# templeblock/audioSignalProcess

Hardware: AMD Instinct MI355X
Metric: audio frames/sec (10 ms @16 kHz) Wiener NS (higher is better)
Workload: dtype f32

## Files before the change

### audiosignalprocess_amd/csrc/ns_kernels1.hip

```cpp
#include <hip/hip_runtime.h>

#include <type_traits>

#include "handoff.h"
#include "ns_device.h"
#include "ns_layout.h"
#include "ns_pair_fft.h"
#include "ns_step.h"

namespace {
using namespace asphandoff;
using namespace aspns_dev;
using namespace aspns_pair;

__device__ __forceinline__ unsigned long long ns_cu_tag() {
  const unsigned hw = __builtin_amdgcn_s_getreg((7 << 11) | (8 << 6) | 4);
  const unsigned xcc = __builtin_amdgcn_s_getreg((3 << 11) | (0 << 6) | 20);
  return (unsigned long long)((xcc << 8) | hw);
}

constexpr int NS3 = 3;

template <typename V>
__device__ __forceinline__ V ns_in_vgpr(V x) {
// ... 98 lines not shown
  }
  __device__ __forceinline__ void image_fill(int lane, const float4 (&v)[kImgVec4]) const {
#pragma unroll
    for (int i = 0; i < kImgVec4; ++i)
      *reinterpret_cast<lds_f32x4*>(img + i * 256 + 4 * lane) = f32x4v{v[i].x, v[i].y, v[i].z, v[i].w};
  }
  __device__ __forceinline__ void image_write_back(int lane) const {
#pragma unroll
    for (int i = 0; i < kImgVec4; ++i) {
      const f32x4v v = *reinterpret_cast<const lds_f32x4*>(img + i * 256 + 4 * lane);
      sc1_store4(rs, lane * 16, i * 1024, make_float4(v.x, v.y, v.z, v.w));
    }
  }
};

template <bool IMG>
struct ScalarRow {
  lds_f32* row;
  static constexpr int kTrk0 = aspns::S_TAIL0 + aspns::V_LQ0, kTrk1 = aspns::S_TAIL0 + aspns::V_DEN2;
  static constexpr bool in_image(int k) { return IMG && k >= aspns::S_OVERDRIVE && !(k >= kTrk0 && k <= kTrk1); }
  __device__ __forceinline__ explicit ScalarRow(float* image) : row((lds_f32*)image + aspns::kOffScalars) {}
  template <int K>
  __device__ __forceinline__ float f(float sv) const {
    if constexpr (in_image(K)) return row[K];
    else return __int_as_float(__builtin_amdgcn_readlane(__float_as_int(sv), K));
  }
  template <int K, int N>
  __device__ __forceinline__ void ld(float sv, float (&v)[N]) const {
    static_assert((N == 2 || N == 4) && K % N == 0 && in_image(K) == in_image(K + N - 1), "one aligned group, one master");
    if constexpr (in_image(K) && N == 2) {
      const f32x2v t = *reinterpret_cast<const lds_f32x2*>(row + K);
      v[0] = t.x; v[1] = t.y;
    } else if constexpr (in_image(K)) {
      const f32x4v t = *reinterpret_cast<const lds_f32x4*>(row + K);
      v[0] = t.x; v[1] = t.y; v[2] = t.z; v[3] = t.w;
    } else {
#pragma unroll
      for (int i = 0; i < N; ++i) v[i] = __int_as_float(__builtin_amdgcn_readlane(__float_as_int(sv), K + i));
    }
  }
  template <int K>
  __device__ __forceinline__ void set(float& sv, float val) const {
    if constexpr (in_image(K)) row[K] = val;
    else sv = setlane_vgpr<K>(sv, val);
  }
  __device__ __forceinline__ void store_owned(int lane, float sv) const {
    if (!IMG || lane < aspns::S_OVERDRIVE || (lane >= kTrk0 && lane <= kTrk1)) row[lane] = sv;
  }
};

struct NsStepScalars {
  int blockInd;
  int updates;
  int counter[3];
  int updateParsFlag;
  int mup3;
  int gainmap;
};
#define NS_STEADY_CONJUNCTS(X, s)                                                                                   \
  X((s).blockInd > NS_END_STARTUP_LONG + 1)                                           \
  X((s).updates >= NS_END_STARTUP_LONG)                                                                              \
  X((s).counter[0] < NS_END_STARTUP_LONG - 1 && (s).counter[1] < NS_END_STARTUP_LONG - 1 &&                           \
    (s).counter[2] < NS_END_STARTUP_LONG - 1)                               \
  X((s).counter[0] >= 0 && (s).counter[1] >= 0 && (s).counter[2] >= 0)                                                \
  X((s).updateParsFlag >= 1)                                                                                         \
  X((s).mup3 > 2)                                                                \
  X((s).gainmap == 1)
__device__ __forceinline__ bool ns_step_is_steady(const NsStepScalars& s) {
  bool steady = true;
#define NS_CONJ_AND(c) steady = steady && (c);
  NS_STEADY_CONJUNCTS(NS_CONJ_AND, s)
#undef NS_CONJ_AND
  return steady;
}
__device__ __forceinline__ void ns_assume_steady(const NsStepScalars& s) {
#define NS_CONJ_ASSUME(c) __builtin_assume(c);
  NS_STEADY_CONJUNCTS(NS_CONJ_ASSUME, s)
#undef NS_CONJ_ASSUME
}

struct NsDiagArgs {
  void* buf;
  int mode;
};

template <bool IO16, bool FLOW, bool DIAG>
__device__ __forceinline__ void ns_frame1_run(float* __restrict__ state, int32_t* __restrict__ hist_all,
                                              const NsTables* __restrict__ T, const float* __restrict__ in,
                                              float* __restrict__ out, int num_streams, int steady_on,
                                              const NsFlowArgs& fa, const NsDiagArgs& dg) {
  [[maybe_unused]] const unsigned long long diag_buf =
      DIAG ? (FLOW ? ns_in_vgpr((unsigned long long)dg.buf) : (unsigned long long)dg.buf) : 0ull;
#ifdef NS1_BUDGET
#define NS_STAMP(k) asm volatile("; NS_PHASE " #k " body %0" : : "n"(ns_body_tag));
#define NS_BUDGET_ASIDE() asm volatile("; NS_PHASE 99 body 3");
#define NS_BUDGET_BACK(k) asm volatile("; NS_PHASE " #k " body %0" : : "n"(ns_body_tag));
#else
  [[maybe_unused]] unsigned stamp_sel = 0;
  if constexpr (DIAG) {
    if (dg.buf != nullptr && dg.mode != 2 && threadIdx.x < 64) {
      if (dg.mode == 1) stamp_sel = 1u;
      else if (FLOW ? blockIdx.x == gridDim.x / 2 : blockIdx.x == 0) stamp_sel = 2u + (FLOW ? fa.steps / 2 : 0u);
    }
  }
#define NS_STAMP(k)                                                                            \
  if constexpr (DIAG) {                                                                        \
    const unsigned stamp_sel_ = __builtin_amdgcn_readfirstlane(stamp_sel);                     \
    if (stamp_sel_ != 0) {                                                                     \
      __builtin_amdgcn_sched_barrier(0);                                                       \
      unsigned long long* const stamps_ = reinterpret_cast<unsigned long long*>(diag_buf);     \
      if (stamp_sel_ == 1u) {                                                                  \
        if ((k) == 0 || (k) == 1 || (k) == 14 || (k) == 15)                                    \
          stamps_[blockIdx.x * 4 + ((k) == 0 ? 0 : (k) == 1 ? 1 : (k) == 14 ? 2 : 3)] =       \
              __builtin_amdgcn_s_memrealtime() | ((k) == 0 ? ns_cu_tag() << 48 : 0ull);       \
      } else if (stamp_sel_ == 2u + flow_j) {                                                  \
        stamps_[k] = __builtin_amdgcn_s_memtime();                                             \
      }                                                                                        \
      __builtin_amdgcn_sched_barrier(0);                                                       \
    }                                                                                          \
  }
#define NS_BUDGET_ASIDE()
#define NS_BUDGET_BACK(k)
#endif
  unsigned flow_j = 0, flow_end = 1, flow_slot = 0;
  [[maybe_unused]] unsigned diag_steps = 0;
  [[maybe_unused]] constexpr int ns_body_tag = 0;
  if constexpr (FLOW) {
    flow_j = blockIdx.y * fa.walk;
    flow_end = flow_j + fa.walk < fa.steps ? flow_j + fa.walk : fa.steps;
    flow_slot = ((unsigned)fa.slot0 + flow_j) % (unsigned)fa.ring;
  } else {
    NS_STAMP(0)
  }
  __shared__ __align__(16) float2 lds[4][130];
  __shared__ __align__(16) float tabs[3 * 64 * 4 + 32 * 4 * 2];
  __shared__ __align__(16) float wins[kAnal];
  __shared__ __align__(16) double exp2s[64];
  __shared__ __align__(16) double2 logts[128];
  __shared__ __align__(16) float imgs[FLOW ? 4 : 1][FLOW ? kImgDwords : 4];
  const int tid = threadIdx.x;
  const float4* tab_src = tid < 192 ? reinterpret_cast<const float4*>(&T->tw[0][0][0]) + tid
                                    : reinterpret_cast<const float4*>(&T->spl[0][0][0]) + (tid - 192);
  const float4 tab_v = *tab_src;
  const float4 win_v = reinterpret_cast<const float4*>(T->window)[tid & 63];
  const double exp2_v = T->exp2_64[tid & 63];
  const double2 logt_v = reinterpret_cast<const double2*>(T->logtab)[tid & 127];
  const int lane = tid & 63;
  const int diagbits = T->diag[lane];
  const int wv = __builtin_amdgcn_readfirstlane(tid >> 6);
  float2* tile = lds[wv];
  const int lam = lane >> 1, h = lane & 1;
  const int g = lam >> 4, q = lam & 15;
  const int binA = q + 64 * g + 16 * h;
  const uint32_t gmask = g ? 0x80000000u : 0u;
  const int stream_raw = blockIdx.x * 4 + wv;
  bool wave_live = stream_raw < num_streams;
  const int stream = wave_live ? stream_raw : num_streams - 1;
  float* __restrict__ st = state + (size_t)stream * kStreamDwords;
  int32_t* __restrict__ hist = hist_all + (size_t)stream * kHistDwords;
  const StateAcc<FLOW> sa(st, FLOW ? imgs[wv] : nullptr);
  float* outj = out;
  auto diag_flush_steps = [&]() __attribute__((always_inline)) {
    if constexpr (DIAG) {
      unsigned* const counts = reinterpret_cast<unsigned*>(diag_buf);
      if (dg.mode == 2 && ns_cold(lane) == 0) {
        atomicAdd(counts + 2 * stream, diag_steps & 0xffffu);
        atomicAdd(counts + 2 * stream + 1, diag_steps >> 16);
      }
    }
  };

  float sv;
  constexpr bool ROW_IMG = FLOW && !DIAG;
  const ScalarRow<ROW_IMG> srow(imgs[FLOW ? wv : 0]);
#define SC_I(k) __builtin_amdgcn_readlane(__float_as_int(sv), (k))
#define SC_F(k) srow.template f<(k)>(sv)
#define SC_SET_I(k, val) sv = writelane_bits<(k)>(sv, (int)(val))
#define SC_SET_F(k, val) srow.template set<(k)>(sv, (val))
  static_assert(S_COUNTER1 == S_COUNTER0 + 1 && S_COUNTER2 == S_COUNTER0 + 2, "the three counters: consecutive lanes");
  float4 s4;
  float2 carryA, carryB;
  float4 s4in = make_float4(0.f, 0.f, 0.f, 0.f);
  const size_t frame_uni = (size_t)stream * kBlockL;
  auto flow_load_in = [&](unsigned slot) __attribute__((always_inline)) {
    const int lane_c = ns_cold(lane);
    const unsigned frame_lane = 4u * (unsigned)((lane_c < 24 ? 24 : lane_c) - 24);
    const float* base = IO16 ? reinterpret_cast<const float*>(reinterpret_cast<const short*>(in + (size_t)slot * fa.per) + frame_uni)
                             : in + (size_t)slot * fa.per + frame_uni;
    s4in = load_frame4<IO16>(base, frame_lane);
  };
  auto flow_head = [&](auto head_c) __attribute__((always_inline)) {
    [[maybe_unused]] constexpr int ns_body_tag = decltype(head_c)::value;
    NS_STAMP(0)
    outj = out + (size_t)flow_slot * fa.per;
    const int lane_c = ns_cold(lane);
    const float4 ha = sa.ld4(kOffAnaHist, 4 * (lane_c < 24 ? lane_c : 23));
    const bool hsel = lane_c < 24;
    s4.x = hsel ? ha.x : s4in.x;
    s4.y = hsel ? ha.y : s4in.y;
    s4.z = hsel ? ha.z : s4in.z;
    s4.w = hsel ? ha.w : s4in.w;
    const int q2_c = lane_c & 30;
    carryA = sa.ld2(kOffSynt, q2_c + 32 * (lane_c & 1));
    carryB = sa.ld2(kOffSynt, q2_c + 64);
  };
  [[maybe_unused]] float4 img_v[FLOW ? kImgVec4 : 1];
  if constexpr (FLOW) {
    flow_load_in(flow_slot);
    if (wave_live) wave_live = handoff_wait(fa.hand, fa.want + flow_j, stream, lane);
    if (wave_live) sa.image_request(lane, img_v);
  } else {
    sv = st[kOffScalars + lane];
    float* hbuf = st + kOffAnaHist;
    if (!IO16) {
      const float* src = lane < 24 ? hbuf + 4 * lane : in + (size_t)stream * kBlockL + 4 * (lane - 24);
      s4 = *reinterpret_cast<const float4*>(src);
    } else {
      const int lh = lane < 24 ? lane : 23, li = lane < 24 ? 24 : lane;
      const float4 ha = *reinterpret_cast<const float4*>(hbuf + 4 * lh);
      const short* in16 = reinterpret_cast<const short*>(in) + (size_t)stream * kBlockL + 4 * (li - 24);
      const short4 a = *reinterpret_cast<const short4*>(in16);
      const bool hsel = lane < 24;
      s4.x = hsel ? ha.x : (float)a.x;
      s4.y = hsel ? ha.y : (float)a.y;
      s4.z = hsel ? ha.z : (float)a.z;
      s4.w = hsel ? ha.w : (float)a.w;
    }
    carryA = *reinterpret_cast<const float2*>(st + kOffSynt + 2 * q + 32 * h);
    carryB = *reinterpret_cast<const float2*>(st + kOffSynt + 2 * q + 64);
  }

  reinterpret_cast<float4*>(tabs)[tid] = tab_v;
  if (tid < 64) exp2s[tid] = exp2_v;
  if (tid < 128) logts[tid] = logt_v;
  if (tid >= 192) reinterpret_cast<float4*>(wins)[tid - 192] = win_v;
  if constexpr (FLOW) {
    if (wave_live) sa.image_fill(lane, img_v);
  }
  __syncthreads();
  if (!wave_live) return;
  if constexpr (FLOW) {
    sv = sa.ld1(kOffScalars, lane);
    flow_head(std::integral_constant<int, 3>{});
  }
  const float* tws = tabs;
  const float* spls = tabs + 3 * 64 * 4;
  const PairFftLane fl = pair_fft_lane(lane, diagbits);

#define LOADV(dst, f)                                                                          \
  {                                                                                            \
    const float2 v2_ = sa.ld2(kOffVec + (f)*kVecStride, 2 * lane);                             \
    dst[0] = v2_.x; dst[1] = v2_.y;                                                            \
  }
#define LOADT(dst, f) dst[2] = SC_F(S_TAIL0 + (f));
#define LOAD3(dst, f) LOADV(dst, f) LOADT(dst, f)
#define STORE3(f, srcv)                                                                        \
  {                                                                                            \
    sa.st2(kOffVec + (f)*kVecStride, 2 * lane, srcv[0], srcv[1]);                              \
    SC_SET_F(S_TAIL0 + (f), srcv[2]);                                                          \
  }
#define STORE3_HOT(f, srcv)                                                                    \
  {                                                                                            \
    sa.st2(kOffVec + (f)*kVecStride, 2 * lane, srcv[0], srcv[1]);                              \
    if constexpr (!ROW_IMG) SC_SET_F(S_TAIL0 + (f), srcv[2]);                                  \
  }
#define NS_NEXT_FRAME()                                                                        \
  if constexpr (FLOW) {                                                                        \
    flow_slot = flow_slot + 1u == (unsigned)fa.ring ? 0u : flow_slot + 1u;                     \
    if (flow_j + 1u < flow_end) flow_load_in(flow_slot);                                       \
  }
#define NS_STREAM_DONE(head_tag)                                                               \
  if constexpr (FLOW) {                                                                        \
    [[maybe_unused]] constexpr int ns_body_tag = head_tag;  \
    const bool walk_done_ = flow_j + 1u >= flow_end;                                           \
    if (walk_done_) {                                                                          \
      NS_BUDGET_ASIDE()                                                                        \
      const int lane_w_ = ns_cold(lane);                                                       \
      srow.store_owned(lane_w_, sv);                                                           \
      lds_sync1();                                                                             \
      sa.image_write_back(lane_w_);                                                            \
      handoff_drain();                                                                         \
    }                                                                                          \
    NS_STAMP(16)                                                                               \
    if (walk_done_) {                                                                          \
      NS_BUDGET_ASIDE()                                                                        \
      diag_flush_steps();                                                                      \
      if (lane == 0) handoff_publish(fa.hand.seq + stream, fa.want + flow_j);                  \
      return;                                                                                  \
    }                                                                                          \
    ++flow_j;                                                                                  \
    lds_sync1();                                                                               \
    NS_BUDGET_BACK(16)                                                                         \
    flow_head(std::integral_constant<int, head_tag>{});                                        \
    continue;                                                                                  \
  } else {                                                                                     \
    diag_flush_steps();                                                                        \
    return;                                                                                    \
  }

  constexpr bool CARRY = FLOW;
  [[maybe_unused]] f32x2 carry_stsa = {0.f, 0.f};
  [[maybe_unused]] float carry_stsa_tail = 0.f;
  [[maybe_unused]] bool carry_ok = false;
  for (;;) {
    NS_BUDGET_BACK(0)
    float LQ[3][NS3], DEN[3][NS3], quant[NS3];
    float smooth[NS3], noisePrev[NS3], magnPrevA[NS3], logLrt[NS3], avgPause[NS3];


    const float4 w4 = *reinterpret_cast<const float4*>(wins + 4 * lane);
    const float wx0 = w4.x * s4.x, wx1 = w4.y * s4.y, wx2 = w4.z * s4.z, wx3 = w4.w * s4.w;
    float epart = wx0 * wx0;
    epart += wx1 * wx1;
    epart += wx2 * wx2;
    epart += wx3 * wx3;
    const float energy1 = wave_sum_bcast(epart);

    {
      const int lane_c = ns_cold(lane);
      if (lane_c >= 40) sa.st4(kOffAnaHist, 4 * (lane_c - 40), s4);
    }

    if (energy1 == 0.0f) {
      NS_BUDGET_ASIDE()
      float* y = IO16 ? reinterpret_cast<float*>(reinterpret_cast<short*>(outj) + (size_t)stream * kBlockL)
                      : outj + (size_t)stream * kBlockL;
      NS_NEXT_FRAME()
      const int lane_c = ns_cold(lane);
      float2 o01 = make_float2(0.f, 0.f);
      if (lane_c < 48) o01 = sa.ld2(kOffSynt, 2 * lane_c);
      __builtin_amdgcn_fence(__ATOMIC_ACQ_REL, "wavefront");
      store2p<IO16>(y, 2 * lane_c, sat16p(o01.x), sat16p(o01.y));
      if (lane_c < 16) store2p<IO16>(y, 128 + 2 * lane_c, 0.f, 0.f);
      if (lane_c < 48) sa.st2(kOffSynt, 2 * lane_c, 0.f, 0.f);
      NS_STREAM_DONE(3)
    }
    NS_BUDGET_BACK(0)

    LOADV(LQ[0], V_LQ0) LOADV(LQ[1], V_LQ1) LOADV(LQ[2], V_LQ2)
    LOADV(DEN[0], V_DEN0) LOADV(DEN[1], V_DEN1) LOADV(DEN[2], V_DEN2)
    LOADV(quant, V_QUANT)
    NS_STAMP(1)
    *reinterpret_cast<float4*>(&tile[2 * lane]) = make_float4(wx0, wx1, wx2, wx3);
    lds_sync1();
    f32x2 er, ei;
    {
      f32x2 ea, eb;
      cft128_passes1(tile, tws, fl, lane, ea, eb);
      radix2_tail1(ea, eb, gmask, false, er, ei);
    }
    real_split1(tile, spls, lane, er, ei, false);

    NS_STAMP(2)
    if constexpr (!CARRY) LOADV(magnPrevA, V_MAGNPREV_A)
    LOADV(logLrt, V_LOGLRT) LOADV(avgPause, V_AVGPAUSE)
    if constexpr (!CARRY) LOADV(smooth, V_SMOOTH)
    LOADV(noisePrev, V_NOISEPREV)

    float re[NS3], im[NS3], magn[NS3];
    re[0] = er.x;
    im[0] = ei.x;
    re[1] = er.y;
    im[1] = ei.y;
    re[2] = lane_bcast(ei.x, 0);
    im[2] = 0.f;
    if (lane == 0) im[0] = 0.f;
    {
      float m2[2] = {re[0] * re[0] + im[0] * im[0], re[1] * re[1] + im[1] * im[1]}, rt[2];
      fsqrt_n<2>(m2, rt);
      magn[0] = rt[0] + 1.f;
      magn[1] = rt[1] + 1.f;
    }
    if (lane == 0) magn[0] = fabsf(re[0]) + 1.f;
    magn[2] = fabsf(re[2]) + 1.f;

#define SUM3(v) (wave_sum_bcast(v[0] + v[1]) + v[2])

    NsStepScalars ss;
    ss.blockInd = SC_I(S_BLOCKIND) + 1;
    ss.updates = SC_I(S_UPDATES);
    ss.counter[0] = SC_I(S_COUNTER0);
    ss.counter[1] = SC_I(S_COUNTER1);
    ss.counter[2] = SC_I(S_COUNTER2);
    ss.updateParsFlag = SC_I(S_MUP0);
    ss.mup3 = SC_I(S_MUP3);
    ss.gainmap = SC_I(S_GAINMAP);
    const bool step_steady = steady_on != 0 && ns_step_is_steady(ss);
    static_assert(kCntTerms == NS_END_STARTUP_LONG + 1, "one entry per counter value");
    float cterm[3][3];
    auto load_cterms = [&]() __attribute__((always_inline)) {
#pragma unroll
      for (int s = 0; s < 3; ++s) {
        typedef const __attribute__((address_space(4))) float cfloat_k;
        const unsigned n = (unsigned)ss.counter[s] < (unsigned)NS_END_STARTUP_LONG ? (unsigned)ss.counter[s]
                                                                                   : (unsigned)NS_END_STARTUP_LONG;
#pragma unroll
        for (int j = 0; j < 3; ++j) cterm[s][j] = *(cfloat_k*)(&T->cnt_terms[n][j]);
      }
    };
    auto step_rest = [&](auto steady_c) __attribute__((always_inline)) {
      constexpr bool STEADY = decltype(steady_c)::value;
      [[maybe_unused]] constexpr int ns_body_tag = STEADY ? 1 : 2;
      if constexpr (STEADY) ns_assume_steady(ss);
      if constexpr (DIAG) diag_steps += STEADY ? 1u : 0x10000u;
      load_cterms();
      const int blockInd = ss.blockInd;
      float priorSpeechProb;
      const int gainmap = ss.gainmap;

      float noise[NS3], prevStsa[NS3];
      const int updateParsFlag = ss.updateParsFlag;
      int updates = ss.updates;
      int counter[3] = {ss.counter[0], ss.counter[1], ss.counter[2]};

      float snrLocPost[NS3], snrLocPrior[NS3];
      auto snr_tail = [&](float noise2) __attribute__((always_inline)) {
        const float q2t = fdiv(magn[2], noise2 + 0.0001f);
        float previousEstimateStsa;
        if (CARRY && carry_ok) {
          previousEstimateStsa = carry_stsa_tail;
        } else {
          const float q1t = fdiv(magnPrevA[2], noisePrev[2] + 0.0001f);
          previousEstimateStsa = q1t * smooth[2];
        }
        prevStsa[2] = previousEstimateStsa;
        snrLocPost[2] = 0.f;
        if (magn[2] > noise2) snrLocPost[2] = q2t - 1.f;
        snrLocPrior[2] = NS_DD_PR_SNR * previousEstimateStsa + (1.f - NS_DD_PR_SNR) * snrLocPost[2];
      };
      auto load_snr_tails = [&]() __attribute__((always_inline)) {
        static_assert(V_SMOOTH == V_QUANT + 1 && V_MAGNPREV_A == V_NOISEPREV + 1, "row tails read as pairs");
        float t2[2], u2[2];
        srow.template ld<S_TAIL0 + V_QUANT, 2>(sv, t2);
        srow.template ld<S_TAIL0 + V_NOISEPREV, 2>(sv, u2);
        quant[2] = t2[0]; smooth[2] = t2[1];
        noisePrev[2] = u2[0]; magnPrevA[2] = u2[1];
      };
      float lmagn[NS3];
      [[maybe_unused]] float lt1_tail = 0.f;
      if constexpr (STEADY) {
        load_snr_tails();
        snr_tail(quant[2]);
        const float xs[NS3] = {magn[0], magn[1], lane == 1 ? 1.f + 2.f * snrLocPrior[2] : magn[2]};
        log_f32_via_tab_n<NS3>(xs, lmagn, logts);
        lt1_tail = lane_bcast(lmagn[2], 1);
        lmagn[2] = lane_bcast(lmagn[2], 0);
      } else {
        log_f32_via_tab_n<NS3>(magn, lmagn, logts);
      }
      LOADT(avgPause, V_AVGPAUSE)

      NS_STAMP(3)
      float signalEnergy, sumMagn, flatNum, avgPauseMean;
      {
        float p_se = (re[0] * re[0] + im[0] * im[0]) + (re[1] * re[1] + im[1] * im[1]);
        float p_sm = magn[0] + magn[1];
        float p_fl = lane == 0 ? lmagn[1] : lmagn[0] + lmagn[1];
        float p_ap = avgPause[0] + avgPause[1];
        wave_sums_bcast(p_se, p_sm, p_fl, p_ap);
        signalEnergy = p_se + (re[2] * re[2] + im[2] * im[2]);
        sumMagn = p_sm + magn[2];
        flatNum = p_fl + lmagn[2];
        avgPauseMean = p_ap + avgPause[2];
        signalEnergy = DIV129(signalEnergy);
      }

      NS_STAMP(4)
      if constexpr (!STEADY) load_snr_tails();
      if (updates < NS_END_STARTUP_LONG) updates++;
      bool quant_new = false;
      constexpr int kLqLane = S_TAIL0 + V_LQ0, kDenLane = S_TAIL0 + V_DEN0;
      static_assert(V_LQ1 == V_LQ0 + 1 && V_LQ2 == V_LQ0 + 2 && V_DEN1 == V_DEN0 + 1 && V_DEN2 == V_DEN0 + 2 &&
                    kDenLane == kLqLane + 3 && kLqLane / 16 == (kDenLane + 2) / 16,
                    "the tracker tails: three + three consecutive lanes of one DPP row");
      float lqT = sv, denT = dpp_move<0x103>(sv);
      {
#define NS_LANES3_F(j) __int_as_float(lanes3_bits<kLqLane>(__float_as_int(cterm[0][j]), __float_as_int(cterm[1][j]), \
                                                           __float_as_int(cterm[2][j])))
        const float cntv = NS_LANES3_F(0), cnt1v = NS_LANES3_F(1), rcnt1v = NS_LANES3_F(2);
#undef NS_LANES3_F
        tracker_step1(lqT, denT, lmagn[2], cntv, cnt1v, rcnt1v);
      }
#pragma unroll
      for (int s = 0; s < 3; ++s) {
        {
          const float cnt = cterm[s][0], cnt1 = cterm[s][1], rcnt1 = cterm[s][2];
          f32x2 lq = {LQ[s][0], LQ[s][1]}, den = {DEN[s][0], DEN[s][1]};
          tracker_step2(lq, den, f32x2{lmagn[0], lmagn[1]}, cnt, cnt1, rcnt1);
          LQ[s][0] = lq.x; LQ[s][1] = lq.y;
          DEN[s][0] = den.x; DEN[s][1] = den.y;
        }
        if (counter[s] >= NS_END_STARTUP_LONG) {
          counter[s] = 0;
          if (updates >= NS_END_STARTUP_LONG) {
            LQ[s][2] = lane_bcast(lqT, kLqLane + s);
            exp_f32_via_f64_n<NS3>(LQ[s], quant, exp2s);
            quant_new = true;
          }
        }
        counter[s]++;
      }
      if (updates < NS_END_STARTUP_LONG) {
        LQ[2][2] = lane_bcast(lqT, kLqLane + 2);
        exp_f32_via_f64_n<NS3>(LQ[2], quant, exp2s);
        quant_new = true;
      }
#pragma unroll
      for (int k = 0; k < NS3; ++k) noise[k] = quant[k];
#pragma unroll
      for (int s = 0; s < 3; ++s) sa.st2(kOffVec + (V_LQ0 + s) * kVecStride, 2 * lane, LQ[s][0], LQ[s][1]);
#pragma unroll
      for (int s = 0; s < 3; ++s) sa.st2(kOffVec + (V_DEN0 + s) * kVecStride, 2 * lane, DEN[s][0], DEN[s][1]);
      sv = mergelanes_vgpr<(7ull << kLqLane)>(sv, lqT);
      sv = mergelanes_vgpr<(7ull << kDenLane)>(sv, dpp_move<0x113>(denT));
      if (quant_new) STORE3(V_QUANT, quant)

      NS_STAMP(5)
// ... 211 lines not shown
        priorSpeechProb = ns_prior_update(priorSpeechProb, pm, ns_prior_indicator(lane_bcast(th, 0)),
                                          ns_prior_indicator(lane_bcast(th, 1)), ns_prior_indicator(lane_bcast(th, 2)));
      }
      float probSpeech[NS3];
      {
        const float gainPrior = fdiv(1.f - priorSpeechProb, priorSpeechProb + 0.0001f);
        {
          float pd[NS3];
          const float ones[NS3] = {1.f, 1.f, 1.f};
#pragma unroll
          for (int k = 0; k < NS3; ++k) {
            float invLrt = ev[k];
            invLrt = (float)gainPrior * invLrt;
            pd[k] = 1.f + invLrt;
          }
          fdiv3(ones, pd, probSpeech);
        }
      }

      NS_STAMP(10)
      {
        const int srcA = q > 0 ? lane - 2 : (h ? 30 + 32 * g : 31);
        const int srcB = q > 0 ? lane - 2 : (h ? 30 + 32 * g : 31 + 32 * g);
        const bool a_from1 = q == 0 && h == 0;
        const bool b_from1 = q > 0 || h == 1;
        const float a0 = __shfl(probSpeech[0], srcA, 64), a1 = __shfl(probSpeech[1], srcA, 64);
        const float b0 = __shfl(probSpeech[0], srcB, 64), b1 = __shfl(probSpeech[1], srcB, 64);
        float prevProb[NS3];
        prevProb[0] = a_from1 ? a1 : a0;
        prevProb[1] = b_from1 ? b1 : b0;
        prevProb[2] = lane_bcast(probSpeech[1], 63);
        {
          const F3 np(noisePrev), mg(magn), ps(probSpeech), ap(avgPause);
          const F3 x = (1.f - ps) * mg + ps * np;
          const F3 uS = NS_SPEECH_UPDATE * np + (1.f - NS_SPEECH_UPDATE) * x;
          const F3 uN = NS_NOISE_UPDATE * np + (1.f - NS_NOISE_UPDATE) * x;
          B3 oldSpeech = gt3(F3(prevProb), F3(NS_PROB_RANGE));
          oldSpeech.v[0] = oldSpeech.v[0] && lane != 0;
          const F3 uOld = sel3(oldSpeech, uS, uN);
          const F3 uNew = sel3(gt3(ps, F3(NS_PROB_RANGE)), uS, uN);
          min3(uOld, uNew).store(noise);
          sel3(lt3(ps, F3(NS_PROB_RANGE)), ap + NS_GAMMA_PAUSE * (mg - ap), ap).store(avgPause);
        }
      }
      STORE3_HOT(V_LOGLRT, logLrt) STORE3_HOT(V_AVGPAUSE, avgPause)
      STORE3_HOT(V_MAGNPREV_A, magn)

      NS_STAMP(11)
      float initMagn[NS3], pnoise[NS3];
      if (startup) {
        if constexpr (FLOW) {
          handoff_drain();
          const int lane2_c = 2 * ns_cold(lane);
          const float2 im_ = sa.ld2(kOffVec + V_INITMAGN * kVecStride, lane2_c);
          const float2 pn_ = sa.ld2(kOffVec + V_PARAMNOISE * kVecStride, lane2_c);
          initMagn[0] = im_.x; initMagn[1] = im_.y;
          pnoise[0] = pn_.x; pnoise[1] = pn_.y;
          LOADT(initMagn, V_INITMAGN) LOADT(pnoise, V_PARAMNOISE)
#pragma unroll
          for (int k = 0; k < NS3; ++k) initMagn[k] += magn[k];
          sa.st2(kOffVec + V_INITMAGN * kVecStride, lane2_c, initMagn[0], initMagn[1]);
          SC_SET_F(S_TAIL0 + V_INITMAGN, initMagn[2]);
        } else {
          LOAD3(initMagn, V_INITMAGN)
          LOAD3(pnoise, V_PARAMNOISE)
#pragma unroll
          for (int k = 0; k < NS3; ++k) initMagn[k] += magn[k];
          STORE3(V_INITMAGN, initMagn)
        }
      }
      float overdrive, denoiseBound;
      {
        static_assert(S_DENOISEBOUND == S_OVERDRIVE + 1, "scalars read as a pair");
        float t2[2];
        srow.template ld<S_OVERDRIVE, 2>(sv, t2);
        overdrive = t2[0]; denoiseBound = t2[1];
      }
      float gainv[NS3];
      float gq1[NS3], gq2[NS3], snrP[NS3];
      {
        float gd1[NS3], gd2[NS3];
#pragma unroll
        for (int k = 0; k < NS3; ++k) gd1[k] = noise[k] + 0.0001f;
        fdiv3(magn, gd1, gq1);
#pragma unroll
        for (int k = 0; k < NS3; ++k) {
          float currentEstimateStsa = 0.f;
          if (magn[k] > noise[k]) currentEstimateStsa = gq1[k] - 1.f;
          snrP[k] = NS_DD_PR_SNR * prevStsa[k] + (1.f - NS_DD_PR_SNR) * currentEstimateStsa;
          gd2[k] = overdrive + snrP[k];
        }
        fdiv3(snrP, gd2, gq2);
      }
#pragma unroll
      for (int k = 0; k < NS3; ++k) {
        float gg = fmin_raw(fmax_raw(gq2[k], denoiseBound), 1.f);
        if (startup) {
          float tmp = (initMagn[k] - overdrive * pnoise[k]);
          tmp /= (initMagn[k] + 0.0001f);
          if (tmp < denoiseBound) tmp = denoiseBound;
          if (tmp > 1.f) tmp = 1.f;
          gg *= (blockInd);
          tmp *= (NS_END_STARTUP_SHORT - blockInd);
          gg += tmp;
          gg /= (NS_END_STARTUP_SHORT);
        }
        gainv[k] = gg;
        re[k] *= gg;
        im[k] *= gg;
      }
      if constexpr (CARRY) {
        carry_stsa = f32x2{gq1[0], gq1[1]} * f32x2{gainv[0], gainv[1]};
        carry_stsa_tail = gq1[2] * gainv[2];
        carry_ok = true;
      }
      STORE3_HOT(V_SMOOTH, gainv)
      STORE3_HOT(V_NOISEPREV, noise)
      auto commit_floats = [&]() __attribute__((always_inline)) {
        if constexpr (ROW_IMG) {
          SC_SET_F(S_TAIL0 + V_LOGLRT, logLrt[2]);
          SC_SET_F(S_TAIL0 + V_AVGPAUSE, avgPause[2]);
          SC_SET_F(S_TAIL0 + V_MAGNPREV_A, magn[2]);
          SC_SET_F(S_TAIL0 + V_SMOOTH, gainv[2]);
          SC_SET_F(S_TAIL0 + V_NOISEPREV, noise[2]);
        }
        SC_SET_F(S_SIGNALENERGY, signalEnergy);
        SC_SET_F(S_SUMMAGN, sumMagn);
        if (startup) {
          SC_SET_F(S_WHITE, whiteNoiseLevel);
          SC_SET_F(S_PINKNUM, pinkNoiseNumerator);
          SC_SET_F(S_PINKEXP, pinkNoiseExp);
        }
        if (window_closed) {
          SC_SET_F(S_PMP0, pm.p0);
          SC_SET_F(S_PMP1, pm.p1);
          SC_SET_F(S_PMP3, pm.p3);
          SC_SET_F(S_PMP4, pm.p4);
          SC_SET_F(S_PMP5, pm.p5);
          SC_SET_F(S_PMP6, pm.p6);
        }
        SC_SET_F(S_FD0, fd0);
        SC_SET_F(S_FD3, fd3);
        SC_SET_F(S_FD4, fd4);
        SC_SET_F(S_FD5, fd5);
        SC_SET_F(S_FD6, fd6);
        SC_SET_F(S_PRIORSPEECHPROB, priorSpeechProb);
      };
      if constexpr (ROW_IMG) {
        if (lane == 0) commit_floats();
      }

      NS_STAMP(12)
      NS_NEXT_FRAME()
      er = f32x2{re[0], re[1]};
      ei = f32x2{im[0], im[1]};
      if (lane == 0) ei.x = re[2];
      real_split1(tile, spls, lane, er, ei, true);
      lds_sync1();
      {
        const int base = 64 * g + q + 16 * h;
        float* tf = reinterpret_cast<float*>(tile);
        tf[2 * base] = er.x;
        tf[2 * base + 1] = ei.x;
        tf[2 * base + 64] = er.y;
        tf[2 * base + 65] = ei.y;
      }
      lds_sync1();
      f32x2 tr, ti;
      {
        f32x2 ea, eb;
        cft128_passes1(tile, tws, fl, lane, ea, eb);
        radix2_tail1(ea, eb, gmask, true, tr, ti);
      }
      const float td0 = tr.x * (2.f / kAnal), td1 = ti.x * (2.f / kAnal);
      const float td2 = tr.y * (2.f / kAnal), td3s = ti.y * (2.f / kAnal);

      NS_STAMP(13)
      float factor = 1.f;
      if (gainmap == 1 && blockInd > NS_END_STARTUP_LONG) {
        float e2 = td0 * td0;
        e2 += td1 * td1;
        e2 += td2 * td2;
        e2 += td3s * td3s;
        factor = ns_gain_factor(wave_sum_bcast(e2), energy1, denoiseBound, priorSpeechProb);
      }

      {
        float* y = IO16 ? reinterpret_cast<float*>(reinterpret_cast<short*>(outj) + (size_t)stream * kBlockL)
                        : outj + (size_t)stream * kBlockL;
        __builtin_amdgcn_fence(__ATOMIC_ACQ_REL, "wavefront");
        const int nA = 2 * ns_cold(binA), nB = nA + 64;
        const float2 wA = *reinterpret_cast<const float2*>(wins + nA);
        const float2 wB = *reinterpret_cast<const float2*>(wins + nB);
        const float cA0 = g == 0 ? carryA.x : 0.f, cA1 = g == 0 ? carryA.y : 0.f;
        const float cB0 = (g == 0 && h == 0) ? carryB.x : 0.f, cB1 = (g == 0 && h == 0) ? carryB.y : 0.f;
        const float oA0 = cA0 + factor * (wA.x * td0), oA1 = cA1 + factor * (wA.y * td1);
        const float oB0 = cB0 + factor * (wB.x * td2), oB1 = cB1 + factor * (wB.y * td3s);
        if (nA >= 160) {
          sa.st2(kOffSynt, nA - 160, oA0, oA1);
        } else {
          store2p<IO16>(y, nA, sat16p(oA0), sat16p(oA1));
        }
        if (nB >= 160) {
          sa.st2(kOffSynt, nB - 160, oB0, oB1);
        } else {
          store2p<IO16>(y, nB, sat16p(oB0), sat16p(oB1));
        }
      }

      NS_STAMP(14)
      if constexpr (STEADY) {
        sv = addlanes_bits<(1ull << S_BLOCKIND) | (7ull << S_COUNTER0), 1ull << S_MUP3>(sv);
      } else {
        SC_SET_I(S_UPDATES, updates);
        SC_SET_I(S_COUNTER0, counter[0]);
        SC_SET_I(S_COUNTER1, counter[1]);
        SC_SET_I(S_COUNTER2, counter[2]);
        SC_SET_I(S_MUP0, mup0);
        SC_SET_I(S_MUP3, mup3);
        SC_SET_I(S_BLOCKIND, blockInd);
      }
      if constexpr (!ROW_IMG) commit_floats();
    };
    if (__builtin_expect(step_steady, 1)) step_rest(std::true_type{});
    else step_rest(std::false_type{});
    if constexpr (!FLOW) sa.st1(kOffScalars, lane, sv);
    NS_STAMP(15)
    NS_STREAM_DONE(0)
  }
#undef NS_STREAM_DONE
#undef NS_NEXT_FRAME
#undef NS_STAMP
#undef NS_BUDGET_ASIDE
#undef NS_BUDGET_BACK
#undef SC_I
#undef SC_F
#undef SC_SET_I
#undef SC_SET_F
#undef LOAD3
#undef LOADV
#undef LOADT
#undef STORE3
#undef STORE3_HOT
#undef SUM3
}

template <bool IO16, bool FLOW>
__global__ __launch_bounds__(256, 4) void ns_frame1_kernel(float* __restrict__ state,
                                                           int32_t* __restrict__ hist_all,
                                                           const NsTables* __restrict__ T,
                                                           const float* __restrict__ in,
                                                           float* __restrict__ out,
                                                           int num_streams, int steady_on, NsFlowArgs fa) {
  ns_frame1_run<IO16, FLOW, false>(state, hist_all, T, in, out, num_streams, steady_on, fa, NsDiagArgs{nullptr, 0});
}

template <bool FLOW>
__global__ __launch_bounds__(256, 4) void ns_frame1_diag_kernel(float* __restrict__ state,
                                                                int32_t* __restrict__ hist_all,
                                                                const NsTables* __restrict__ T,
                                                                const float* __restrict__ in,
                                                                float* __restrict__ out,
                                                                int num_streams, int steady_on, NsFlowArgs fa,
                                                                NsDiagArgs dg) {
  ns_frame1_run<false, FLOW, true>(state, hist_all, T, in, out, num_streams, steady_on, fa, dg);
}

__global__ void debug_tanh_wave_kernel(unsigned start, unsigned count, unsigned* n_bad, unsigned* bad_bits,
                                       const NsTables* __restrict__ T) {
  const unsigned i = blockIdx.x * blockDim.x + threadIdx.x;
  if (i >= count) return;
  const float x = __uint_as_float(start + i);
  const float a = tanh_f32_via_f64_wave(x, T->exp2_64), b = (float)tanh((double)x);
  const bool same = (__float_as_uint(a) == __float_as_uint(b)) || (a != a && b != b);
  if (!same) {
    const unsigned k = atomicAdd(n_bad, 1u);
    if (k < 64) bad_bits[k] = start + i;
  }
}

}

namespace aspns {

hipError_t launch_debug_tanh_wave(unsigned start, unsigned count, unsigned* n_bad, unsigned* bad_bits,
                                  const NsTables* T, hipStream_t s) {
  hipLaunchKernelGGL(debug_tanh_wave_kernel, dim3((count + 255u) / 256u), dim3(256), 0, s, start, count, n_bad, bad_bits, T);
  return hipGetLastError();
}

hipError_t launch_ns_frame1(bool io16, float* state, int32_t* hist, const NsTables* T,
                            const float* in, float* out, int num_streams, hipStream_t s, int steady_on,
                            unsigned long long* stamps, int stamp_mode, unsigned* step_counts) {
  const dim3 grid((num_streams + 3) / 4), block(256);
  const NsFlowArgs none = {{nullptr, nullptr}, 0u, 0, 1, 0u, 1u, 1u};
  if (stamps != nullptr || step_counts != nullptr) {
    if (io16) return hipErrorInvalidValue;
    const NsDiagArgs dg = {stamps != nullptr ? (void*)stamps : (void*)step_counts, stamps != nullptr ? (stamp_mode != 0 ? 1 : 0) : 2};
    hipLaunchKernelGGL((ns_frame1_diag_kernel<false>), grid, block, 0, s, state, hist, T, in, out, num_streams,
                       steady_on, none, dg);
  } else if (io16)
    hipLaunchKernelGGL((ns_frame1_kernel<true, false>), grid, block, 0, s, state, hist, T, in, out,
                       num_streams, steady_on, none);
  else
    hipLaunchKernelGGL((ns_frame1_kernel<false, false>), grid, block, 0, s, state, hist, T, in, out,
                       num_streams, steady_on, none);
  return hipGetLastError();
}

hipError_t launch_ns_frame1_flow(bool io16, float* state, int32_t* hist, const NsTables* T,
                                 const float* in, float* out, int num_streams, hipStream_t s,
                                 unsigned* seq, unsigned* abort_w, unsigned want, int steps, int walk, int slot0,
                                 int ring, size_t per, int steady_on, unsigned long long* stamps,
                                 unsigned* step_counts) {
  walk = walk < 1 ? 1 : (walk > steps ? steps : walk);
  const int gx = ((num_streams + 3) / 4 + 7) / 8 * 8;
  const dim3 grid(gx, (steps + walk - 1) / walk), block(256);
  const NsFlowArgs fa = {{seq, abort_w}, want, slot0, ring, (unsigned)per, (unsigned)steps, (unsigned)walk};
  if (stamps != nullptr || step_counts != nullptr) {
    if (io16) return hipErrorInvalidValue;
    const NsDiagArgs dg = {stamps != nullptr ? (void*)stamps : (void*)step_counts, stamps != nullptr ? 0 : 2};
    hipLaunchKernelGGL((ns_frame1_diag_kernel<true>), grid, block, 0, s, state, hist, T, in, out, num_streams,
                       steady_on, fa, dg);
  } else if (io16)
    hipLaunchKernelGGL((ns_frame1_kernel<true, true>), grid, block, 0, s, state, hist, T, in, out,
                       num_streams, steady_on, fa);
  else
    hipLaunchKernelGGL((ns_frame1_kernel<false, true>), grid, block, 0, s, state, hist, T, in, out,
// ... 6 lines not shown
```

### audiosignalprocess_amd/csrc/ns_pair_fft.h

```cpp
#pragma once
#include <hip/hip_runtime.h>

#include "ns_device.h"

namespace aspns_pair {
using namespace aspns_dev;

__device__ __forceinline__ void lds_sync1() {
  __builtin_amdgcn_fence(__ATOMIC_RELEASE, "wavefront");
  __builtin_amdgcn_wave_barrier();
  __builtin_amdgcn_fence(__ATOMIC_ACQUIRE, "wavefront");
}

struct PairFftLane {
  float s;
  float kap0, kap1, kap2;
  bool h;
};
__device__ __forceinline__ PairFftLane pair_fft_lane(int lane, int diagbits) {
  PairFftLane L;
  L.h = (lane & 1) != 0;
  L.s = L.h ? -1.0f : 1.0f;
  L.kap0 = (float)(diagbits & 1);
  L.kap1 = (float)((diagbits >> 1) & 1);
  L.kap2 = (float)((diagbits >> 2) & 1);
  return L;
}

template <int ROT>
__device__ __forceinline__ f32x2 rot_add(float k, f32x2 a) {
  f32x2 kk = {k, k}, r;
  if (ROT > 0)
    asm("v_pk_fma_f32 %0, %1, %2, %2 op_sel:[0,1,0] op_sel_hi:[0,0,1] neg_lo:[0,1,0]" : "=v"(r) : "v"(kk), "v"(a));
  else
    asm("v_pk_fma_f32 %0, %1, %2, %2 op_sel:[0,1,0] op_sel_hi:[0,0,1] neg_hi:[0,1,0]" : "=v"(r) : "v"(kk), "v"(a));
  return r;
}
__device__ __forceinline__ f32x2 cmul_pk(f32x2 a, f32x2 t) {
  const f32x2 p1 = a.xx * t;
  const f32x2 p2 = a.yy * t.yx;
  f32x2 r;
  asm("v_pk_add_f32 %0, %1, %2 neg_lo:[0,1]" : "=v"(r) : "v"(p1), "v"(p2));
  return r;
}

__device__ __forceinline__ void half_bfly(f32x2 c0, f32x2 c1, f32x2 c2, f32x2 c3, const PairFftLane& L,
                                          float kap, float4 tw, f32x2& first, f32x2& second) {
  const f32x2 ss = {L.s, L.s};
  const f32x2 u = __builtin_elementwise_fma(ss, c1, c0);
  const f32x2 v = __builtin_elementwise_fma(ss, c3, c2);
  const f32x2 v2 = {L.h ? -v.y : v.x, L.h ? v.x : v.y};
  const f32x2 p = u + v2, m = u - v2;
  first = cmul_pk(rot_add<+1>(kap, p), f32x2{tw.x, tw.y});
  second = cmul_pk(rot_add<-1>(kap, m), f32x2{tw.z, tw.w});
}

__device__ __forceinline__ f32x2 ldsc(const float2* t, int i) {
  const float2 v = t[i];
  return f32x2{v.x, v.y};
}
__device__ __forceinline__ void stsc(float2* t, int i, f32x2 v) { t[i] = make_float2(v.x, v.y); }

__device__ __forceinline__ void cft128_passes1(float2* tile, const float* tws, const PairFftLane& L,
                                               int lane, f32x2& oA, f32x2& oB) {
  const int b = lane >> 1;
  const int hh = lane & 1;
  f32x2 f, s;
  {
    const int rb = (int)(__brev((unsigned)b) >> 27);
    const float4 tw = *reinterpret_cast<const float4*>(tws + (0 * 64 + lane) * 4);
    half_bfly(ldsc(tile, rb), ldsc(tile, rb + 64), ldsc(tile, rb + 32), ldsc(tile, rb + 96), L, L.kap0, tw, f, s);
    lds_sync1();
    stsc(tile, 4 * b + hh, f);
    stsc(tile, 4 * b + 2 + hh, s);
  }
  lds_sync1();
  {
    const int base = 16 * (b >> 2) + (b & 3);
    const float4 tw = *reinterpret_cast<const float4*>(tws + (1 * 64 + lane) * 4);
    half_bfly(ldsc(tile, base), ldsc(tile, base + 4), ldsc(tile, base + 8), ldsc(tile, base + 12), L, L.kap1, tw, f, s);
    lds_sync1();
    stsc(tile, base + 4 * hh, f);
    stsc(tile, base + 8 + 4 * hh, s);
  }
  lds_sync1();
  {
    const int base = 64 * (b >> 4) + (b & 15);
    const float4 tw = *reinterpret_cast<const float4*>(tws + (2 * 64 + lane) * 4);
    half_bfly(ldsc(tile, base), ldsc(tile, base + 16), ldsc(tile, base + 32), ldsc(tile, base + 48), L, L.kap2, tw, oA, oB);
  }
}

__device__ __forceinline__ float tail_combine(float v, uint32_t gmask) {
  const unsigned u = __float_as_uint(v);
  const auto r = __builtin_amdgcn_permlane32_swap(u, u, false, false);
  return __uint_as_float(r[0]) + xorf(__uint_as_float(r[1]), gmask);
}
__device__ __forceinline__ void radix2_tail1(f32x2 a, f32x2 b, uint32_t gmask, bool backward, f32x2& er, f32x2& ei) {
  const float ar = tail_combine(a.x, gmask), ai = tail_combine(a.y, gmask);
  const float br = tail_combine(b.x, gmask), bi = tail_combine(b.y, gmask);
  er = f32x2{ar, br};
  ei = backward ? f32x2{-ai, -bi} : f32x2{ai, bi};
}

__device__ __forceinline__ void real_split1(float2* tile, const float* spls, int lane, f32x2& er, f32x2& ei,
                                            bool backward) {
  const int b = lane >> 1, h = lane & 1;
  const bool hi = b >= 16;
  const int base = 64 * (b >> 4) + (b & 15) + 16 * h;
  float* tf = reinterpret_cast<float*>(tile);
  lds_sync1();
  tf[2 * base] = er.x;
  tf[2 * base + 1] = ei.x;
  tf[2 * base + 64] = er.y;
  tf[2 * base + 65] = ei.y;
  lds_sync1();
  const float sg = hi ? -1.0f : 1.0f;
  const f32x2 sgs = {sg, sg};
  const int pi0 = 2 * (128 - base);
  const f32x2 per = {tf[pi0], tf[pi0 - 64]}, pei = {tf[pi0 + 1], tf[pi0 - 63]};
  const float* wp = spls + (b * 4 + h) * 2;
  const f32x2 wr = {wp[0], wp[4]}, wi = {wp[1], wp[5]};
  const f32x2 xr = sgs * (er - per), xi = ei + pei;
  f32x2 rr, ri;
  if (!backward) {
    const f32x2 yr = wr * xr - wi * xi, yi = wr * xi + wi * xr;
    rr = __builtin_elementwise_fma(-sgs, yr, er);
    ri = ei - yi;
    if (lane == 0) {
      rr.x = er.x + ei.x;
      ri.x = er.x - ei.x;
    }
  } else {
    const f32x2 yr = wr * xr + wi * xi, yi = wr * xi - wi * xr;
    rr = __builtin_elementwise_fma(-sgs, yr, er);
    ri = yi - ei;
    if (lane == 0) {
      const float hh = 0.5f * (er.x - ei.x);
      rr.x = er.x - hh;
      ri.x = -hh;
    }
  }
  er = rr;
  ei = ri;
}

template <bool IO16>
__device__ __forceinline__ void store2p(float* y, int idx, float a, float b) {
  if (IO16) {
    short2 v;
    const float kMaxRound = 32767 - 0.5f, kMinRound = -32768 + 0.5f;
    v.x = a > 0 ? (a >= kMaxRound ? (short)32767 : (short)(a + 0.5f))
                : (a <= kMinRound ? (short)-32768 : (short)(a - 0.5f));
    v.y = b > 0 ? (b >= kMaxRound ? (short)32767 : (short)(b + 0.5f))
                : (b <= kMinRound ? (short)-32768 : (short)(b - 0.5f));
    *reinterpret_cast<short2*>(reinterpret_cast<short*>(y) + idx) = v;
  } else {
    *reinterpret_cast<float2*>(y + idx) = make_float2(a, b);
  }
}

__device__ __forceinline__ float sat16p(float x) {
  return x > 32767 ? 32767 : (x < -32768 ? -32768 : x);
}

template <int K>
__device__ __forceinline__ float writelane_bits(float row, int bits) {
  int r = __float_as_int(row);
  const int u = __builtin_amdgcn_readfirstlane(bits);
  asm("v_writelane_b32 %0, %1, %2" : "+v"(r) : "s"(u), "n"(K));
  return __int_as_float(r);
}
template <int K>
__device__ __forceinline__ float setlane_vgpr(float row, float val) {
  const unsigned long long mask = 1ull << K;
  asm("v_cndmask_b32 %0, %0, %1, %2" : "+v"(row) : "v"(val), "s"(mask));
  return row;
}
template <unsigned long long MASK>
__device__ __forceinline__ float mergelanes_vgpr(float row, float val) {
  const unsigned long long mask = MASK;
  asm("v_cndmask_b32 %0, %0, %1, %2" : "+v"(row) : "v"(val), "s"(mask));
  return row;
}
template <unsigned long long UP, unsigned long long DOWN>
__device__ __forceinline__ float addlanes_bits(float row) {
  int r = __float_as_int(row);
  const unsigned long long up = UP, down = DOWN;
  asm("v_addc_co_u32_e64 %0, vcc, 0, %0, %1\n\tv_subb_co_u32_e64 %0, vcc, %0, 0, %2" : "+v"(r) : "s"(up), "s"(down) : "vcc");
  return __int_as_float(r);
}
template <int K>
__device__ __forceinline__ int lanes3_bits(int a, int b, int c) {
  return __float_as_int(writelane_bits<K + 1>(writelane_bits<K>(__int_as_float(c), a), b));
}

}
```

Measured before the change: 485.4 million.

## Fuse radix-2 FFT tail into real-split and pack split arithmetic in complex pairs

Removes the separate permlane32 radix-2 tail before the forward real split. The split now loads the partner half-wave values from LDS and folds the final butterfly into it. The backward path writes its split results straight into the tile for the inverse FFT, dropping a separate store-and-sync round. Split arithmetic is also rewritten to packed (re,im) pairs using inline v_pk_add/v_pk_fma with negation modifiers. The risk is subtle sign and index mistakes in the rewritten butterfly/split mapping, and more LDS reads replacing cross-lane swaps.

```diff
diff --git a/audiosignalprocess_amd/csrc/ns_kernels1.hip b/audiosignalprocess_amd/csrc/ns_kernels1.hip
--- a/audiosignalprocess_amd/csrc/ns_kernels1.hip
+++ b/audiosignalprocess_amd/csrc/ns_kernels1.hip
@@ -274,7 +274,6 @@
   const int lam = lane >> 1, h = lane & 1;
   const int g = lam >> 4, q = lam & 15;
   const int binA = q + 64 * g + 16 * h;
-  const uint32_t gmask = g ? 0x80000000u : 0u;
   const int stream_raw = blockIdx.x * 4 + wv;
   bool wave_live = stream_raw < num_streams;
   const int stream = wave_live ? stream_raw : num_streams - 1;
@@ -431,11 +430,13 @@
 
 
     const float4 w4 = *reinterpret_cast<const float4*>(wins + 4 * lane);
-    const float wx0 = w4.x * s4.x, wx1 = w4.y * s4.y, wx2 = w4.z * s4.z, wx3 = w4.w * s4.w;
-    float epart = wx0 * wx0;
-    epart += wx1 * wx1;
-    epart += wx2 * wx2;
-    epart += wx3 * wx3;
+    const f32x2 wx01 = f32x2{w4.x, w4.y} * f32x2{s4.x, s4.y}, wx23 = f32x2{w4.z, w4.w} * f32x2{s4.z, s4.w};
+    const f32x2 sq01 = wx01 * wx01, sq23 = wx23 * wx23;
+    const float wx0 = wx01.x, wx1 = wx01.y, wx2 = wx23.x, wx3 = wx23.y;
+    float epart = sq01.x;
+    epart += sq01.y;
+    epart += sq23.x;
+    epart += sq23.y;
     const float energy1 = wave_sum_bcast(epart);
 
     {
@@ -465,13 +466,12 @@
     NS_STAMP(1)
     *reinterpret_cast<float4*>(&tile[2 * lane]) = make_float4(wx0, wx1, wx2, wx3);
     lds_sync1();
-    f32x2 er, ei;
+    f32x2 z0, z1;
     {
       f32x2 ea, eb;
       cft128_passes1(tile, tws, fl, lane, ea, eb);
-      radix2_tail1(ea, eb, gmask, false, er, ei);
-    }
-    real_split1(tile, spls, lane, er, ei, false);
+      tail_split_fwd1(tile, spls, lane, ea, eb, z0, z1);
+    }
 
     NS_STAMP(2)
     if constexpr (!CARRY) LOADV(magnPrevA, V_MAGNPREV_A)
@@ -480,11 +480,11 @@
     LOADV(noisePrev, V_NOISEPREV)
 
     float re[NS3], im[NS3], magn[NS3];
-    re[0] = er.x;
-    im[0] = ei.x;
-    re[1] = er.y;
-    im[1] = ei.y;
-    re[2] = lane_bcast(ei.x, 0);
+    re[0] = z0.x;
+    im[0] = z0.y;
+    re[1] = z1.x;
+    im[1] = z1.y;
+    re[2] = lane_bcast(z0.y, 0);
     im[2] = 0.f;
     if (lane == 0) im[0] = 0.f;
     {
@@ -1002,28 +1002,21 @@
 
       NS_STAMP(12)
       NS_NEXT_FRAME()
-      er = f32x2{re[0], re[1]};
-      ei = f32x2{im[0], im[1]};
-      if (lane == 0) ei.x = re[2];
-      real_split1(tile, spls, lane, er, ei, true);
+      z0 = f32x2{re[0], lane == 0 ? re[2] : im[0]};
+      z1 = f32x2{re[1], im[1]};
+      split_bwd1(tile, spls, lane, z0, z1);
       lds_sync1();
-      {
-        const int base = 64 * g + q + 16 * h;
-        float* tf = reinterpret_cast<float*>(tile);
-        tf[2 * base] = er.x;
-        tf[2 * base + 1] = ei.x;
-        tf[2 * base + 64] = er.y;
-        tf[2 * base + 65] = ei.y;
-      }
-      lds_sync1();
-      f32x2 tr, ti;
+      f32x2 tA, tB;
       {
         f32x2 ea, eb;
         cft128_passes1(tile, tws, fl, lane, ea, eb);
-        radix2_tail1(ea, eb, gmask, true, tr, ti);
-      }
-      const float td0 = tr.x * (2.f / kAnal), td1 = ti.x * (2.f / kAnal);
-      const float td2 = tr.y * (2.f / kAnal), td3s = ti.y * (2.f / kAnal);
+        const float sg = g ? -1.0f : 1.0f;
+        const f32x2 sgs = {sg, sg};
+        tA = tail_swap1(ea, sgs);
+        tB = tail_swap1(eb, sgs);
+      }
+      const float td0 = tA.x * (2.f / kAnal), td1 = -tA.y * (2.f / kAnal);
+      const float td2 = tB.x * (2.f / kAnal), td3s = -tB.y * (2.f / kAnal);
 
       NS_STAMP(13)
       float factor = 1.f;
diff --git a/audiosignalprocess_amd/csrc/ns_pair_fft.h b/audiosignalprocess_amd/csrc/ns_pair_fft.h
--- a/audiosignalprocess_amd/csrc/ns_pair_fft.h
+++ b/audiosignalprocess_amd/csrc/ns_pair_fft.h
@@ -91,58 +91,84 @@
   }
 }
 
-__device__ __forceinline__ float tail_combine(float v, uint32_t gmask) {
-  const unsigned u = __float_as_uint(v);
-  const auto r = __builtin_amdgcn_permlane32_swap(u, u, false, false);
-  return __uint_as_float(r[0]) + xorf(__uint_as_float(r[1]), gmask);
-}
-__device__ __forceinline__ void radix2_tail1(f32x2 a, f32x2 b, uint32_t gmask, bool backward, f32x2& er, f32x2& ei) {
-  const float ar = tail_combine(a.x, gmask), ai = tail_combine(a.y, gmask);
-  const float br = tail_combine(b.x, gmask), bi = tail_combine(b.y, gmask);
-  er = f32x2{ar, br};
-  ei = backward ? f32x2{-ai, -bi} : f32x2{ai, bi};
-}
-
-__device__ __forceinline__ void real_split1(float2* tile, const float* spls, int lane, f32x2& er, f32x2& ei,
-                                            bool backward) {
+__device__ __forceinline__ f32x2 tail_swap1(f32x2 a, f32x2 sgs) {
+  const unsigned ux = __float_as_uint(a.x), uy = __float_as_uint(a.y);
+  const auto rx = __builtin_amdgcn_permlane32_swap(ux, ux, false, false);
+  const auto ry = __builtin_amdgcn_permlane32_swap(uy, uy, false, false);
+  const f32x2 lo = {__uint_as_float(rx[0]), __uint_as_float(ry[0])};
+  const f32x2 hi = {__uint_as_float(rx[1]), __uint_as_float(ry[1])};
+  return __builtin_elementwise_fma(sgs, hi, lo);
+}
+
+template <bool BACKWARD>
+__device__ __forceinline__ f32x2 split_elem(f32x2 e, f32x2 pe, f32x2 w, f32x2 c1) {
+  f32x2 d, r;
+  asm("v_pk_add_f32 %0, %1, %2 neg_lo:[0,1]" : "=v"(d) : "v"(e), "v"(pe));
+  const f32x2 x = c1 * d;
+  const f32x2 p1 = w.xx * x;
+  const f32x2 p2 = w.yy * x.yx;
+  f32x2 y;
+  if (!BACKWARD) {
+    asm("v_pk_add_f32 %0, %1, %2 neg_lo:[0,1]" : "=v"(y) : "v"(p1), "v"(p2));
+    asm("v_pk_fma_f32 %0, %1, %2, %3 neg_lo:[1,0,0] neg_hi:[1,0,0]" : "=v"(r) : "v"(c1), "v"(y), "v"(e));
+  } else {
+    asm("v_pk_add_f32 %0, %1, %2 neg_hi:[0,1]" : "=v"(y) : "v"(p1), "v"(p2));
+    asm("v_pk_fma_f32 %0, %1, %2, %3 neg_lo:[1,0,0] neg_hi:[0,0,1]" : "=v"(r) : "v"(c1), "v"(y), "v"(e));
+  }
+  return r;
+}
+
+__device__ __forceinline__ void tail_split_fwd1(float2* tile, const float* spls, int lane, f32x2 oA, f32x2 oB,
+                                                f32x2& z0, f32x2& z1) {
   const int b = lane >> 1, h = lane & 1;
   const bool hi = b >= 16;
-  const int base = 64 * (b >> 4) + (b & 15) + 16 * h;
-  float* tf = reinterpret_cast<float*>(tile);
-  lds_sync1();
-  tf[2 * base] = er.x;
-  tf[2 * base + 1] = ei.x;
-  tf[2 * base + 64] = er.y;
-  tf[2 * base + 65] = ei.y;
+  const int e0 = 64 * (b >> 4) + (b & 15) + 16 * h;
+  lds_sync1();
+  stsc(tile, e0, oA);
+  stsc(tile, e0 + 32, oB);
   lds_sync1();
   const float sg = hi ? -1.0f : 1.0f;
   const f32x2 sgs = {sg, sg};
-  const int pi0 = 2 * (128 - base);
-  const f32x2 per = {tf[pi0], tf[pi0 - 64]}, pei = {tf[pi0 + 1], tf[pi0 - 63]};
-  const float* wp = spls + (b * 4 + h) * 2;
-  const f32x2 wr = {wp[0], wp[4]}, wi = {wp[1], wp[5]};
-  const f32x2 xr = sgs * (er - per), xi = ei + pei;
-  f32x2 rr, ri;
-  if (!backward) {
-    const f32x2 yr = wr * xr - wi * xi, yi = wr * xi + wi * xr;
-    rr = __builtin_elementwise_fma(-sgs, yr, er);
-    ri = ei - yi;
-    if (lane == 0) {
-      rr.x = er.x + ei.x;
-      ri.x = er.x - ei.x;
-    }
-  } else {
-    const f32x2 yr = wr * xr + wi * xi, yi = wr * xi - wi * xr;
-    rr = __builtin_elementwise_fma(-sgs, yr, er);
-    ri = yi - ei;
-    if (lane == 0) {
-      const float hh = 0.5f * (er.x - ei.x);
-      rr.x = er.x - hh;
-      ri.x = -hh;
-    }
-  }
-  er = rr;
-  ei = ri;
+  const int x0 = e0 ^ 64;
+  const f32x2 eA = __builtin_elementwise_fma(sgs, oA, ldsc(tile, x0));
+  const f32x2 eB = __builtin_elementwise_fma(sgs, oB, ldsc(tile, x0 + 32));
+  const int p0 = (128 - e0) & 63, p1 = (96 - e0) & 63;
+  const float sp0 = lane == 32 ? -1.0f : -sg;
+  const f32x2 sp0s = {sp0, sp0};
+  const f32x2 pA = __builtin_elementwise_fma(sp0s, ldsc(tile, p0 + 64), ldsc(tile, p0));
+  const f32x2 pB = __builtin_elementwise_fma(-sgs, ldsc(tile, p1 + 64), ldsc(tile, p1));
+  const float2* wp = reinterpret_cast<const float2*>(spls) + (b * 4 + h);
+  const f32x2 c1 = {sg, 1.0f};
+  z0 = split_elem<false>(eA, pA, ldsc(wp, 0), c1);
+  z1 = split_elem<false>(eB, pB, ldsc(wp, 2), c1);
+  if (lane == 0) {
+    z0.x = eA.x + eA.y;
+    z0.y = eA.x - eA.y;
+  }
+}
+
+__device__ __forceinline__ void split_bwd1(float2* tile, const float* spls, int lane, f32x2 z0, f32x2 z1) {
+  const int b = lane >> 1, h = lane & 1;
+  const bool hi = b >= 16;
+  const int e0 = 64 * (b >> 4) + (b & 15) + 16 * h;
+  lds_sync1();
+  stsc(tile, e0, z0);
+  stsc(tile, e0 + 32, z1);
+  lds_sync1();
+  const float sg = hi ? -1.0f : 1.0f;
+  const f32x2 pA = ldsc(tile, 128 - e0), pB = ldsc(tile, 96 - e0);
+  const float2* wp = reinterpret_cast<const float2*>(spls) + (b * 4 + h);
+  const f32x2 c1 = {sg, 1.0f};
+  f32x2 r0 = split_elem<true>(z0, pA, ldsc(wp, 0), c1);
+  const f32x2 r1 = split_elem<true>(z1, pB, ldsc(wp, 2), c1);
+  if (lane == 0) {
+    const float hh = 0.5f * (z0.x - z0.y);
+    r0.x = z0.x - hh;
+    r0.y = -hh;
+  }
+  lds_sync1();
+  stsc(tile, e0, r0);
+  stsc(tile, e0 + 32, r1);
 }
 
 template <bool IO16>
```

Measured after the change: 487.9 million, median of 3. About the same (+0.5%).
